# i2Nav-WHU/IC-GVINS

Hardware: NVIDIA H100
Metric: frames/sec (KLT+BA) 1280x560 300-feat 10-KF window (higher is better)
Workload: dtype u8/int32 fixed point + f32 (KLT), f64 (BA)

## Files before the change

### ic_gvins_b200/csrc/ba.cu

```cuda
#include <cooperative_groups.h>
#include <dlfcn.h>
#include <unistd.h>
#include <math.h>
#include <nccl.h>
#include <stdlib.h>
#include <string.h>

#include <algorithm>
#include <string>
#include <thread>
#include <vector>

#include "ba_math.cuh"
#include "common.cuh"
#include "geom_core.cuh"

namespace icg {
using namespace bam;
namespace cg = cooperative_groups;

constexpr int BA_SPLIT_W = 4;
constexpr int BA_CHOL_NB = 8;
constexpr int BA_MARG_MAXB = 72;
constexpr int BA_MAX_NODES = 32;
// ... 259 lines not shown
    __syncthreads();
    if (tid == 0) s_last = atomicAdd(D.vis_cnt + (size_t) w * C.K + rn, 1) == D.ref_nrun[(size_t) w * C.K + rn] - 1;
    __syncthreads();
    if (!s_last) return;
    __threadfence();
    if (tid == 0) D.vis_cnt[(size_t) w * C.K + rn] = 0;
    const int PM = C.K * (C.K - 1), P = D.npairs[w];
    const int *pro = D.pair_ro + (size_t) w * PM, *poff = D.part_off + (size_t) w * (PM + 1);
    for (int p = tid; p < P; p += 128)
        if ((pro[p] >> 8) == rn) {
            atomicAdd(&s_np, 1);
            if (p == 0 || (pro[p - 1] >> 8) != rn) s_p0 = p;
        }
    __syncthreads();
    const double *part = D.gpart + (size_t) w * C.GQ * 210;
    double *Mp = lin_Mp(C, D, b, w);
    for (int p = s_p0 + warp; p < s_p0 + s_np; p += 4) {
        const int k0 = poff[p], k1 = poff[p + 1];
        double acc[7];
#pragma unroll
        for (int j = 0; j < 7; j++) acc[j] = lane + 32 * j < 210 ? __ldcg(part + (size_t) k0 * 210 + lane + 32 * j) : 0.0;
        for (int k = k0 + 1; k < k1; k++) {
            double v[7];
#pragma unroll
            for (int j = 0; j < 7; j++) v[j] = lane + 32 * j < 210 ? __ldcg(part + (size_t) k * 210 + lane + 32 * j) : 0.0;
#pragma unroll
            for (int j = 0; j < 7; j++) acc[j] += v[j];
        }
#pragma unroll
        for (int j = 0; j < 7; j++)
            if (lane + 32 * j < 210) Mp[(size_t) p * 210 + lane + 32 * j] = acc[j];
    }
}


__device__ __forceinline__ void gram2_slots(const BaCaps &C, const BaDev &D, int w, int K, short *s_slot) {
    const int PM = C.K * (C.K - 1), P = D.npairs[w];
    const int *pro = D.pair_ro + (size_t) w * PM;
    for (int e = threadIdx.x; e < K * K; e += blockDim.x) s_slot[e] = -1;
    __syncthreads();
    for (int p = threadIdx.x; p < P; p += blockDim.x) s_slot[(pro[p] >> 8) * K + (pro[p] & 255)] = (short) p;
    __syncthreads();
}
__device__ __forceinline__ double gram2_entry(const BaCaps &C, const BaDev &D, int buf, int w, int K, const short *s_slot, int A, int B) {
    const int P = D.npairs[w];
    const double *Mp = lin_Mp(C, D, buf, w);
    const int bA = A < 6 * K ? A / 6 : K, bB = B < 6 * K ? B / 6 : K;
    const int a = A - 6 * bA, b = B - 6 * bB;
    const int ga = 12 + a, gb = 12 + b;
    double sum = 0;
    if (bA == K) {
        const int idx = tri20(ga, gb);
        double s4[4] = {0, 0, 0, 0};
        int p = 0;
        for (; p + 16 <= P; p += 16) {
            double v[16];
#pragma unroll
            for (int u = 0; u < 16; u++) v[u] = Mp[(size_t) (p + u) * 210 + idx];
#pragma unroll
            for (int u = 0; u < 16; u++) s4[u & 3] += v[u];
        }
        for (; p < P; p++) s4[p & 3] += Mp[(size_t) p * 210 + idx];
        sum = (s4[0] + s4[1]) + (s4[2] + s4[3]);
    } else if (bB == K || bB == bA) {
        const int i1 = tri20(a, bB == K ? gb : b), i2 = tri20(6 + a, bB == K ? gb : 6 + b);
        for (int o0 = 0; o0 < K; o0 += 8) {
            double v1[8], v2[8];
#pragma unroll
            for (int u = 0; u < 8; u++) {
                const int o = o0 + u;
                const int p1 = o < K ? s_slot[bA * K + o] : -1, p2 = o < K ? s_slot[o * K + bA] : -1;
                v1[u] = p1 >= 0 ? Mp[(size_t) p1 * 210 + i1] : 0.0;
                v2[u] = p2 >= 0 ? Mp[(size_t) p2 * 210 + i2] : 0.0;
            }
#pragma unroll
            for (int u = 0; u < 8; u++) sum += v1[u], sum += v2[u];
        }
    } else {
        const int p1 = s_slot[bA * K + bB], p2 = s_slot[bB * K + bA];
        if (p1 >= 0) sum += Mp[(size_t) p1 * 210 + tri20(a, 6 + b)];
        if (p2 >= 0) sum += Mp[(size_t) p2 * 210 + tri20(b, 6 + a)];
    }
    return sum;
}

__device__ __forceinline__ double block_sum(double v, double *s_red);
__device__ __forceinline__ double block_max(double v, double *s_red);
__device__ __forceinline__ double *x_inbox(const BaDev &D, int peer, int w, int from);
__device__ __forceinline__ int tri_idx(int A, int B, int ncv);

__device__ __forceinline__ void schur_store(const BaCaps &C, const BaDev &D, int buf, int w, int K, const short *s_slot, int A, int B, double cw) {
    const int NCV = 6 * K + 7;
    const bool nccl = !D.S.split && D.world > 1;
    if (A == NCV && !nccl) return;
    const size_t e = (size_t) w * C.NS * C.NS + (size_t) B * C.NS + A;
    const double hc = !D.S.split && !nccl && B < NCV ? lin_Hc(C, D, buf, w)[(size_t) B * C.NS + A] : 0.0;
    const double cj = gram2_entry(C, D, buf, w, K, s_slot, A, B);
    if (D.S.split) {
        double *P = x_inbox(D, w % D.world, w, D.rank);
        const int TRI = NCV * (NCV + 1) / 2;
        if (B < NCV) {
            P[tri_idx(A, B, NCV)] = cj - cw;
            if (A == B) P[TRI + A] = cj;
        } else {
            P[TRI + NCV + A] = cj;
            P[TRI + 2 * NCV + A] = cw;
        }
    } else if (nccl) {
        const size_t NN = (size_t) C.NCA * C.NCA;
        double *R = D.red + (size_t) w * (2 * NN + 8);
        R[(size_t) A * C.NCA + B] = R[(size_t) B * C.NCA + A] = cj;
        R[NN + (size_t) A * C.NCA + B] = R[NN + (size_t) B * C.NCA + A] = cw;
    } else {
        double *V = D.visv + (size_t) w * 3 * C.NCV;
        if (B < NCV) {
// ... 427 lines not shown
    const double *part = D.cost_part + (size_t) w * (nblk_vis + 1);
    double cand = 0;
    const int nb = (dm.F + 255) / 256;
    for (int b = 0; b < nb; b++) cand += part[b];
    if (D.rank == 0) cand += part[nblk_vis];
    D.red2[(size_t) w * 4 + 3] = cand;
}

__global__ void __launch_bounds__(256) ba_hsum(BaCaps C, BaDev D) {
    const int w = blockIdx.y;
    if (D.st[w].done) return;
    const int K = D.dims[w].K, NCV = 6 * K + 7, nn = NCV + 1;
    const int NN = C.NCA * C.NCA;
    const int t = blockIdx.x * 256 + threadIdx.x;
    if (t >= nn * nn) return;
    const int A = t / nn, B = t - A * nn;
    if (B < A || B >= NCV) return;
    const double *RED = D.red + (size_t) w * (2 * NN + 8);
    const double cj = RED[(size_t) B * C.NCA + A], cw = RED[NN + (size_t) B * C.NCA + A];
    D.Hs[(size_t) w * C.NS * C.NS + (size_t) B * C.NS + A] = lin_Hc(C, D, 0, w)[(size_t) B * C.NS + A] + (cj - cw);
}

constexpr int SOLVE_THREADS = 256;

__device__ __forceinline__ double block_sum(double v, double *s_red) {
    const int tid = threadIdx.x, lane = tid & 31, warp = tid >> 5;
    for (int o = 16; o > 0; o >>= 1) v += __shfl_down_sync(0xffffffffu, v, o);
    __syncthreads();
    if (lane == 0) s_red[warp] = v;
    __syncthreads();
    double t = 0;
    if (tid == 0) {
        for (int k = 0; k < (int) (blockDim.x >> 5); k++) t += s_red[k];
        s_red[32] = t;
    }
    __syncthreads();
    return s_red[32];
}
__device__ __forceinline__ double block_max(double v, double *s_red) {
    const int tid = threadIdx.x, lane = tid & 31, warp = tid >> 5;
    for (int o = 16; o > 0; o >>= 1) v = fmax(v, __shfl_down_sync(0xffffffffu, v, o));
    __syncthreads();
    if (lane == 0) s_red[warp] = v;
    __syncthreads();
    if (tid == 0) {
        double t = 0;
        for (int k = 0; k < (int) (blockDim.x >> 5); k++) t = fmax(t, s_red[k]);
        s_red[32] = t;
    }
    __syncthreads();
    return s_red[32];
}

__global__ void __launch_bounds__(SOLVE_THREADS, 2) ba_solve(BaCaps C, BaDev D) {
    extern __shared__ double sm[];
    const int w = blockIdx.x, tid = threadIdx.x;
    LmState &st = D.st[w];
    if (st.done) return;
#ifdef ICG_BA_PHASE_CLOCKS
    unsigned long long clk_prev = D.clk ? clock64() : 0ull;
#define SOLVE_CLK(k)                                              \
    if (D.clk && w == 0 && tid == 0) {                            \
        const unsigned long long t_ = clock64();                  \
        atomicAdd(&D.clk[k], t_ - clk_prev), atomicAdd(&D.clk[8 + (k)], 1ull); \
        clk_prev = t_;                                            \
    }
#define SOLVE_CLK_NOW() (D.clk ? clock64() : 0ull)
#define SOLVE_CLK_ADD(k, t0)                                      \
    if (D.clk && w == 0 && tid == 0) atomicAdd(&D.clk[k], clock64() - (t0)), atomicAdd(&D.clk[8 + (k)], 1ull);
#else
#define SOLVE_CLK(k)
#define SOLVE_CLK_NOW() 0ull
#define SOLVE_CLK_ADD(k, t0)
#endif
    const WinDims dm = D.dims[w];
    const int K = dm.K, L = dm.L, NCV = 6 * K + 7, N = 15 * K + 7;
    const int f_first = st.first, f_fresh = st.fresh_lin, f_last = st.last_success, f_iter = st.iter;
    const double f_gmax_old = st.gmax;
    (void) f_gmax_old;
    double *s_red = sm;
    double *s_scale = s_red + 40;
    double *s_g = s_scale + C.NS;
    double *s_rhs = s_g + C.NS;
    double *s_d2 = s_rhs + C.NS;
    double *s_diag = s_d2 + C.NS;
    double *S = s_diag + C.NS;
    const int b = st.lin_buf;
    const double *Hc = lin_Hc(C, D, b, w), *gcam = lin_gc(C, D, b, w), *Hs = D.Hs + (size_t) w * C.NS * C.NS;
    const bool sharded = D.world > 1;
    const int NN = C.NCA * C.NCA;
    const double *RED = D.red + (size_t) w * (2 * NN + 8), *V = D.visv + (size_t) w * 3 * C.NCV;
    auto hvis_diag = [&](int a) { return sharded ? RED[(size_t) a * C.NCA + a] : V[a]; };
    auto g_vis = [&](int a) { return sharded ? RED[(size_t) a * C.NCA + NCV] : V[NCV + a]; };
    auto wphig = [&](int a) { return sharded ? RED[NN + (size_t) a * C.NCA + NCV] : V[2 * NCV + a]; };
    const double camw = D.rank == 0 ? 1.0 : 0.0;
    if (tid == 0 && st.need_lin) st.need_lin = 0;
    double *scale_c = D.scale_c + (size_t) w * C.NS;
    const double *hl = lin_hl(C, D, b, w), *gl = lin_gl(C, D, b, w), *scale_l = D.scale_l + (size_t) w * C.L;

    for (int a = tid; a < N; a += SOLVE_THREADS) {
        double g = gcam[a];
        if (a < NCV) g += g_vis(a);
        s_g[a] = g;
        if (f_first) {
            double h = Hc[(size_t) a * C.NS + a] + (a < NCV ? hvis_diag(a) : 0.0);
            scale_c[a] = 1.0 / (1.0 + sqrt(h));
        }
    }
    __syncthreads();
    for (int a = tid; a < N; a += SOLVE_THREADS) s_scale[a] = scale_c[a];
    double gmax_now = st.gmax;
    if (f_fresh) {
        double c, gml;
        if (sharded) {
            c = RED[2 * NN];
            gml = D.redmax[w];
        } else {
            double cs = 0, gq = 0;
            const double *costf = lin_costf(C, D, b, w);
            for (int f = tid; f < dm.F; f += SOLVE_THREADS) cs += costf[f];
            for (int l = tid; l < L; l += SOLVE_THREADS) gq = fmax(gq, fabs(gl[l]));
            c = block_sum(cs, s_red);
            gml = block_max(gq, s_red);
        }
        double gm = 0;
        for (int a = tid; a < N; a += SOLVE_THREADS) gm = fmax(gm, fabs(s_g[a]));
        gm = fmax(block_max(gm, s_red), gml);
        gmax_now = gm;
        if (tid == 0) {
            st.x_cost = c + st.cost_cam[b];
            st.gmax = gm;
            if (f_first) st.initial_cost = st.x_cost;
            st.fresh_lin = 0;
        }
        __syncthreads();
    }
    if (f_first) {
        __syncthreads();
        if (tid == 0) st.first = 0;
    }
    {
        int term = 0;
        if (f_iter >= st.max_iter) term = 1;
        else if (f_last && gmax_now <= 1e-10) term = 2;
        else if (f_last && st.radius <= 1e-32) term = 2;
        if (term) {
            __syncthreads();
            if (tid == 0) st.done = term, st.step_valid = 0;
            return;
        }
    }
    __syncthreads();
    if (tid == 0) st.iter++;
    const double radius = st.radius;
    SOLVE_CLK(0)

    constexpr bool async_fill = true;
    if (async_fill) {
        for (int i = tid >> 5; i < N; i += SOLVE_THREADS / 32) {
            const double *src = (i < NCV ? Hs : Hc) + (size_t) i * C.NS;
            const unsigned dst = (unsigned) __cvta_generic_to_shared(S + i * (i + 1) / 2);
            for (int j = tid & 31; j <= i; j += 32)
                asm volatile("cp.async.ca.shared.global [%0], [%1], 8;" ::"r"(dst + 8u * j), "l"(src + j) : "memory");
        }
        asm volatile("cp.async.commit_group;" ::: "memory");
    }
    for (int a = tid; a < N; a += SOLVE_THREADS) {
        double h = Hc[(size_t) a * C.NS + a] + (a < NCV ? hvis_diag(a) : 0.0);
        double hs = s_scale[a] * s_scale[a] * h;
        s_d2[a] = fmin(fmax(hs, 1e-6), 1e32) / radius;
        double gw = a < NCV ? wphig(a) : 0.0;
        s_rhs[a] = -s_scale[a] * (s_g[a] - gw);
    }
    if (async_fill) asm volatile("cp.async.wait_all;" ::: "memory");
    __syncthreads();
    if (async_fill) {
        for (int i = tid >> 5; i < N; i += SOLVE_THREADS / 32) {
            double *row = S + i * (i + 1) / 2;
            const double si = s_scale[i];
            for (int j = tid & 31; j <= i; j += 32) {
                double v = si * s_scale[j] * row[j];
                if (i == j) v += s_d2[i];
                row[j] = v;
            }
        }
    } else {
        for (int i = tid >> 5; i < N; i += SOLVE_THREADS / 32) {
            constexpr int MAXQ = 16;
            double hv[MAXQ];
            const int nq = i / 32 + 1;
#pragma unroll
            for (int q = 0; q < MAXQ; q++) {
                const int j = (tid & 31) + 32 * q;
                hv[q] = 0;
                if (q < nq && j <= i) hv[q] = (i < NCV ? Hs : Hc)[(size_t) i * C.NS + j];
            }
#pragma unroll
            for (int q = 0; q < MAXQ; q++) {
                const int j = (tid & 31) + 32 * q;
                if (q < nq && j <= i) {
                    double v = s_scale[i] * s_scale[j] * hv[q];
                    if (i == j) v += s_d2[i];
                    S[i * (i + 1) / 2 + j] = v;
                }
            }
        }
    }
    for (int a = tid; a < N; a += SOLVE_THREADS) S[N * (N + 1) / 2 + a] = s_rhs[a];
    __syncthreads();
    SOLVE_CLK(1)
    __shared__ int s_fail;
    if (tid == 0) s_fail = 0;
    __syncthreads();
    const int NR = N + 1;
    for (int J0 = 0; J0 < N; J0 += BA_CHOL_NB) {
        const int nb = min(BA_CHOL_NB, N - J0);
        const int lane = tid & 31, warp = tid >> 5, g = lane >> 2, kk = lane & 3;
        const int ntile = (NR - J0 + 7) / 8;
        const unsigned long long pc0 = SOLVE_CLK_NOW();
        (void) pc0;
        const int cb = J0 + g;
        const double *rb = S + (cb < NR ? cb * (cb + 1) / 2 : 0);
        const bool okb = cb < NR;
// ... 593 lines not shown
        for (int j = 0; j < 15; j++) Lm[i * 15 + j] = 0.5 * (inv[i * 15 + j] + inv[j * 15 + i]);
    for (int j = 0; j < 15; j++) {
        double d = Lm[j * 15 + j];
        for (int k = 0; k < j; k++) d -= Lm[j * 15 + k] * Lm[j * 15 + k];
        if (!(d > 0)) return false;
        d = sqrt(d);
        Lm[j * 15 + j] = d;
        for (int i = j + 1; i < 15; i++) {
            double s = Lm[i * 15 + j];
            for (int k = 0; k < j; k++) s -= Lm[i * 15 + k] * Lm[j * 15 + k];
            Lm[i * 15 + j] = s / d;
        }
    }
    for (int i = 0; i < 15; i++)
        for (int j = 0; j < 15; j++) U[i * 15 + j] = j >= i ? Lm[j * 15 + i] : 0.0;
    return true;
}

template <typename T>
struct HostDev {
    T *h = nullptr, *d = nullptr;
    size_t n = 0;
    int alloc(size_t count) {
        n = count;
        if (cudaMallocHost(&h, sizeof(T) * count) != cudaSuccess) return ICG_ENOMEM;
        if (cudaMalloc(&d, sizeof(T) * count) != cudaSuccess) return ICG_ENOMEM;
        memset(h, 0, sizeof(T) * count);
        return ICG_OK;
    }
    void release() {
        if (h) cudaFreeHost(h);
        if (d) cudaFree(d);
        h = d = nullptr;
    }
    cudaError_t up(cudaStream_t s, size_t count = 0) { return cudaMemcpyAsync(d, h, sizeof(T) * (count ? count : n), cudaMemcpyHostToDevice, s); }
    cudaError_t down(cudaStream_t s, size_t count = 0) { return cudaMemcpyAsync(h, d, sizeof(T) * (count ? count : n), cudaMemcpyDeviceToHost, s); }
};
}

struct icg_ba {
    BaCaps C;
    BaDev D;
    int device = 0;
    cudaStream_t stream = nullptr;
    cudaStream_t stream_cam = nullptr;
    cudaEvent_t ev_fork = nullptr, ev_join = nullptr;
    bool own_stream = false;
    int nblk_vis = 0;
    int cur_windows = 0;
    int cam_threads = 160;
    size_t smem_cam, smem_solve, smem_schur;
    int ld_schur;
    int use_global_S;
    HostDev<WinDims> dims;
    HostDev<LmState> st;
    HostDev<double> pose, mix, ext, rho, imu_blob, imu_U, gnss_blh, gnss_std, lever, pose_prior, pose_prior_sinfo, mix_prior, mix_prior_std, marg_x0,
        marg_H0, marg_b0, marg_c0;
    HostDev<int> f_meta_s, vb_lm0, ref_nrun;
    HostDev<double> f_const_s;
    HostDev<int> lm_off, lm_perm, lm_fidx, gnss_node, marg_type, marg_node, part_off, pair_ro, vis_ord, npairs;
    HostDev<uint8_t> f_active;
    std::vector<void *> dev_only;
    HostDev<double> scratch;
    HostDev<LmState> st_save;
    HostDev<int> cull_counters;
    void *comm = nullptr;
    double *xbuf = nullptr;
    size_t xbuf_doubles = 0;
    int x_world = 0;
    void *ipc_opened[8] = {nullptr, nullptr, nullptr, nullptr, nullptr, nullptr, nullptr, nullptr};
    unsigned long long epoch = 0;
    size_t smem_solve_cam = 0, smem_step_lm = 0;
    bool solve_cam_stage_a = false;
    bool solve_cam_dsm = false;
    size_t smem_solve_cam_dsm = 0;
    int dsm_variant = 0;
    bool prof = false;
    std::vector<cudaEvent_t> prof_ev;
    std::vector<int> prof_tag;
    size_t prof_used = 0;
    int prof_skip = 1;
    double prof_ms[16] = {0};
    long prof_cnt[16] = {0};
    bool marg_ready = false;
    MargDev M;
    HostDev<int> marg_map;
    HostDev<double> marg_oJ0, marg_oe0, marg_oHp, marg_obp;
};

extern "C" {
static void prof_collect(icg_ba *h);
static void prof_print(icg_ba *h);
}

static int dmalloc(icg_ba *h, double **p, size_t n) {
    if (cudaMalloc(p, sizeof(double) * n) != cudaSuccess) {
        set_error("icg_ba_create: cudaMalloc of %zu doubles failed", n);
        return ICG_ENOMEM;
    }
    cudaMemsetAsync(*p, 0, sizeof(double) * n, h->stream);
    h->dev_only.push_back(*p);
    return ICG_OK;
}

namespace {
struct NcclApi {
// ... 88 lines not shown
    }
    {
        int prio_lo = 0, prio_hi = 0;
        ICG_CUDA(cudaDeviceGetStreamPriorityRange(&prio_lo, &prio_hi));
        ICG_CUDA(cudaStreamCreateWithPriority(&h->stream_cam, cudaStreamNonBlocking, prio_hi));
    }
    ICG_CUDA(cudaEventCreateWithFlags(&h->ev_fork, cudaEventDisableTiming));
    ICG_CUDA(cudaEventCreateWithFlags(&h->ev_join, cudaEventDisableTiming));
    h->prof = getenv("ICG_BA_PROFILE") != nullptr;
    if (getenv("ICG_BA_CAM_THREADS")) h->cam_threads = std::min(CAM_THREADS, std::max(128, atoi(getenv("ICG_BA_CAM_THREADS")) & ~31));
    if (h->prof) {
        double *ck = nullptr;
        if (dmalloc(h, &ck, 48) != ICG_OK) return ICG_ENOMEM;
        h->D.clk = (unsigned long long *) ck;
    }
    if (getenv("ICG_BA_PROFILE_SKIP")) h->prof_skip = atoi(getenv("ICG_BA_PROFILE_SKIP"));
    BaCaps &C = h->C;
    max_L = std::max(1, max_L), max_F = std::max(1, max_F);
    C.NW = max_windows, C.K = max_K, C.L = max_L, C.F = max_F, C.G = std::max(1, max_gnss), C.R = std::max(1, max_marg_r);
    C.NCV = 6 * max_K + 7, C.N = 15 * max_K + 7, C.NS = (C.N + 3) & ~3, C.NCA = 4 * ((C.NCV + 1 + 3) / 4);
    C.RJ = (2 * max_F + 31) & ~31, C.LP = (max_L + 31) & ~31;
    C.NVB = (max_F + 127 - max_K) / (128 - max_K) + max_L / 128 + 4 + max_K;
    C.GQ = std::max(1, std::min(max_F, (C.NVB - 2) * (max_K - 1)));
    h->nblk_vis = (max_F + 255) / 256;
    const size_t NW = max_windows;
#define HD(field, count)                                                       \
    if (h->field.alloc(count) != ICG_OK) {                                     \
        set_error("icg_ba_create: allocation of " #field " failed");           \
        return ICG_ENOMEM;                                                     \
    }
    HD(dims, NW) HD(st, NW) HD(pose, NW * C.K * 7) HD(mix, NW * C.K * 9) HD(ext, NW * 8) HD(rho, NW * C.L)
    HD(imu_blob, NW * C.K * ICG_IMU_BLOB_DOUBLES) HD(imu_U, NW * C.K * 225) HD(gnss_blh, NW * C.G * 3) HD(gnss_std, NW * C.G * 3) HD(lever, NW * 3)
    HD(pose_prior, NW * 7) HD(pose_prior_sinfo, NW * 6) HD(mix_prior, NW * 9) HD(mix_prior_std, NW * 9) HD(marg_x0, NW * BA_MARG_MAXB * 9)
    HD(marg_H0, NW * C.R * C.R) HD(marg_b0, NW * C.R) HD(marg_c0, NW)
    HD(lm_off, NW * (C.L + 1)) HD(lm_perm, NW * C.L) HD(lm_fidx, NW * C.F) HD(gnss_node, NW * C.G) HD(marg_type, NW * BA_MARG_MAXB) HD(marg_node, NW * BA_MARG_MAXB) HD(f_active, NW * C.F)
    HD(scratch, 1024) HD(st_save, NW) HD(cull_counters, 2 * NW) HD(f_meta_s, NW * C.F * 4) HD(vb_lm0, NW * C.NVB) HD(ref_nrun, NW * C.K) HD(f_const_s, NW * C.F * 14)
    HD(part_off, NW * ((size_t) C.K * (C.K - 1) + 1)) HD(pair_ro, NW * (size_t) C.K * (C.K - 1)) HD(vis_ord, NW * C.F) HD(npairs, NW)
#undef HD
    BaDev &D = h->D;
    D.rank = 0, D.world = 1;
    D.dims = h->dims.d, D.st = h->st.d, D.pose = h->pose.d, D.mix = h->mix.d, D.ext = h->ext.d, D.rho = h->rho.d;
    D.f_active = h->f_active.d;
    D.part_off = h->part_off.d, D.pair_ro = h->pair_ro.d, D.vis_ord = h->vis_ord.d, D.npairs = h->npairs.d;
    D.f_meta_s = h->f_meta_s.d, D.vb_lm0 = h->vb_lm0.d, D.ref_nrun = h->ref_nrun.d, D.f_const_s = h->f_const_s.d;
    D.lm_off = h->lm_off.d, D.lm_perm = h->lm_perm.d, D.imu_blob = h->imu_blob.d, D.imu_U = h->imu_U.d;
    D.gnss_node = h->gnss_node.d, D.gnss_blh = h->gnss_blh.d, D.gnss_std = h->gnss_std.d, D.lever = h->lever.d;
    D.pose_prior = h->pose_prior.d, D.pose_prior_sinfo = h->pose_prior_sinfo.d, D.mix_prior = h->mix_prior.d, D.mix_prior_std = h->mix_prior_std.d;
    D.marg_type = h->marg_type.d, D.marg_node = h->marg_node.d, D.marg_x0 = h->marg_x0.d, D.marg_H0 = h->marg_H0.d, D.marg_b0 = h->marg_b0.d, D.marg_c0 = h->marg_c0.d;
    int rc = ICG_OK;
#define DM(field, count) \
    if (rc == ICG_OK) rc = dmalloc(h, &D.field, count);
    DM(pose_c, NW * C.K * 7) DM(mix_c, NW * C.K * 9) DM(ext_c, NW * 8) DM(rho_c, NW * C.L)
    DM(pose_0, NW * C.K * 7) DM(mix_0, NW * C.K * 9) DM(ext_0, NW * 8) DM(rho_0, NW * C.L)
    DM(AW[0], NW * C.NCA * C.LP) DM(Mp[0], NW * (size_t) C.K * (C.K - 1) * 210) DM(visv, NW * 3 * C.NCV)
    DM(gpart, NW * (size_t) C.GQ * 210) DM(costf[0], NW * C.F) DM(hl[0], NW * C.L) DM(gl[0], NW * C.L) DM(scale_l, NW * C.L) DM(scale_c, NW * C.NS)
    DM(Hc[0], NW * C.NS * C.NS) DM(gc[0], NW * C.NS) DM(Hs, NW * C.NS * C.NS) DM(cost_part, NW * (h->nblk_vis + 1)) DM(red, NW * (2 * (size_t) C.NCA * C.NCA + 8)) DM(redmax, NW) DM(red2, NW * 4) DM(step_c, NW * C.NS) DM(step_l, NW * C.L)
#undef DM
    if (rc == ICG_OK) rc = dmalloc(h, &D.gnss_std_0, NW * C.G * 3);
    if (rc == ICG_OK) {
        double *cnt = nullptr;
        rc = dmalloc(h, &cnt, (NW * C.K + 1) / 2);
        D.vis_cnt = (int *) cnt;
    }
    if (rc == ICG_OK) {
        double *fa0 = nullptr;
        rc = dmalloc(h, &fa0, (NW * C.F + 7) / 8 + 1);
        D.f_active_0 = (uint8_t *) fa0;
    }
    if (rc != ICG_OK) return rc;
    h->smem_cam = sizeof(double) * ((size_t) C.K * 480 + (size_t) C.G * 24 + 48 + 16 + 2 * (size_t) C.R + 8) + sizeof(int) * (size_t) C.R + 64;
    size_t vec = sizeof(double) * (40 + 5 * (size_t) C.NS);
    size_t packed = sizeof(double) * ((size_t) (C.N + 1) * (C.N + 2) / 2);
    h->use_global_S = (vec + packed > 220 * 1024) ? 1 : 0;
    h->smem_solve = vec + (h->use_global_S ? 0 : packed);
    D.Sglobal = nullptr;
    memset(&D.S, 0, sizeof(D.S));
    if (h->use_global_S) {
        rc = split_setup(h, 0, 1);
        if (rc != ICG_OK) return rc;
    } else {
        ICG_CUDA(raise_dynamic_smem((const void *) ba_solve, (size_t) (h->smem_solve)));
    }
    h->ld_schur = 16 * ((C.NCA + 15) / 16) + 8;
    h->smem_schur = sizeof(double) * std::max((size_t) SCHUR_RCH * h->ld_schur + SCHUR_RCH, (size_t) SCHUR_PASS * 256);
    ICG_CUDA(raise_dynamic_smem((const void *) ba_schur_dmma, (size_t) (h->smem_schur)));
    ICG_CUDA(cudaFuncSetAttribute(ba_schur_dmma, cudaFuncAttributePreferredSharedMemoryCarveout, cudaSharedmemCarveoutMaxShared));
    ICG_CUDA(raise_dynamic_smem((const void *) ba_lin_cam, (size_t) (h->smem_cam)));
    ICG_CUDA(raise_dynamic_smem((const void *) ba_cost_cam, (size_t) (h->smem_cam)));
    ICG_CUDA(raise_dynamic_smem((const void *) ba_lin_vis, LV_SMEM));
    ICG_CUDA(cudaStreamSynchronize(h->stream));
    h->cur_windows = 0;
    return ICG_OK;
}

void icg_ba_destroy(icg_ba *h) {
    if (!h) return;
    cudaSetDevice(h->device);
    if (h->stream) cudaStreamSynchronize(h->stream);
    prof_collect(h);
    prof_print(h);
    for (cudaEvent_t e : h->prof_ev) cudaEventDestroy(e);
    h->dims.release(), h->st.release(), h->pose.release(), h->mix.release(), h->ext.release(), h->rho.release();
    h->imu_blob.release(), h->imu_U.release(), h->gnss_blh.release(), h->gnss_std.release(), h->lever.release(), h->pose_prior.release();
    h->pose_prior_sinfo.release(), h->mix_prior.release(), h->mix_prior_std.release(), h->marg_x0.release(), h->marg_H0.release(), h->marg_b0.release();
    h->marg_c0.release(), h->lm_off.release(), h->lm_perm.release(), h->lm_fidx.release(), h->gnss_node.release();
    h->f_meta_s.release(), h->vb_lm0.release(), h->ref_nrun.release(), h->f_const_s.release(), h->marg_type.release(), h->marg_node.release(), h->f_active.release(), h->scratch.release(), h->st_save.release(), h->cull_counters.release(), h->part_off.release(), h->pair_ro.release(), h->vis_ord.release(), h->npairs.release();
    if (h->comm) nccl_api().CommDestroy((ncclComm_t) h->comm);
    split_release(h);
    if (h->marg_ready) h->marg_map.release(), h->marg_oJ0.release(), h->marg_oe0.release(), h->marg_oHp.release(), h->marg_obp.release();
    for (void *p : h->dev_only) cudaFree(p);
    if (h->stream_cam) cudaStreamSynchronize(h->stream_cam), cudaStreamDestroy(h->stream_cam);
    if (h->ev_fork) cudaEventDestroy(h->ev_fork);
    if (h->ev_join) cudaEventDestroy(h->ev_join);
    if (h->own_stream && h->stream) cudaStreamDestroy(h->stream);
    delete h;
}

int icg_ba_upload(icg_ba *h, int n, const icg_ba_problem *P) {
    if (!h || !P || n < 1 || n > h->C.NW) {
        set_error("icg_ba_upload: bad arguments (n=%d, capacity %d)", n, h ? h->C.NW : 0);
        return ICG_EINVAL;
    }
    ICG_CUDA(cudaSetDevice(h->device));
    const BaCaps &C = h->C;
#define PK_FAIL(code, ...)                          \
    do {                                            \
        char eb_[512];                              \
        snprintf(eb_, sizeof(eb_), __VA_ARGS__);    \
        err = eb_;                                  \
        return code;                                \
    } while (0)
    auto pack_one = [&](int w, std::string &err) -> int {
        const icg_ba_problem &p = P[w];
        if (p.K < 2 || p.K > C.K || p.L < 0 || p.L > C.L || p.F < 0 || p.F > C.F || p.n_imu < 0 || p.n_imu > p.K - 1 || p.n_gnss < 0 || p.n_gnss > C.G ||
// ... 224 lines not shown
        h->prof_ev.push_back(e);
        h->prof_tag.push_back(0);
    }
    h->prof_tag[h->prof_used] = tag;
    cudaEventRecord(h->prof_ev[h->prof_used++], h->stream);
}
static void prof_collect(icg_ba *h) {
    if (!h->prof) return;
    if (h->prof_used && h->prof_skip > 0) {
        h->prof_skip--;
        h->prof_used = 0;
        return;
    }
    for (size_t i = 1; i < h->prof_used; i++) {
        float ms = 0;
        if (cudaEventElapsedTime(&ms, h->prof_ev[i - 1], h->prof_ev[i]) == cudaSuccess) {
            h->prof_ms[h->prof_tag[i]] += ms;
            h->prof_cnt[h->prof_tag[i]]++;
        }
    }
    h->prof_used = 0;
}
static void prof_print(icg_ba *h) {
    if (!h->prof) return;
    double tot = 0;
    for (int t = 0; t < 16; t++) tot += h->prof_ms[t];
    fprintf(stderr, "[icg_ba profile] handle %p, %d windows: stage totals over all recorded LM sequences (ms, mean us, share)\n", (void *) h, h->cur_windows);
    for (int t = 0; t < 16; t++)
        if (h->prof_cnt[t])
            fprintf(stderr, "  %-28s %9.3f ms  %8.1f us  %5.1f %%\n", PROF_NAMES[t], h->prof_ms[t], 1e3 * h->prof_ms[t] / h->prof_cnt[t], 100.0 * h->prof_ms[t] / tot);
    if (h->D.clk) {
        unsigned long long ck[48];
        if (cudaMemcpy(ck, h->D.clk, sizeof(ck), cudaMemcpyDeviceToHost) == cudaSuccess) {
            static const char *cn[6] = {"factor evaluation", "prior product + cost", "zero H_c", "prior blocks", "IMU J^T J", "GNSS / prior diagonals"};
            fprintf(stderr, "[icg_ba profile] ba_lin_cam phases of window 0 (SM cycles per call, mean):\n");
            for (int k = 0; k < 6; k++)
                if (ck[24 + k]) fprintf(stderr, "  %-28s %9.0f cycles\n", cn[k], (double) ck[16 + k] / (double) ck[24 + k]);
            if (h->D.S.split) {
                static const char *sn_l2[6] = {"per panel: stage B operand", "per panel: warp 0 tile + factor", "per panel: tiles + barrier 1", "per panel: row solve + barrier 2", "whole factorisation", ""};
                static const char *sn_dsm[6] = {"assembly", "per panel: warp 0 tile + factor", "per panel: until block barrier", "per panel: row solve + cl. barrier", "whole factorisation", "backward substitution"};
                const char **sn = h->solve_cam_dsm ? sn_dsm : sn_l2;
                fprintf(stderr, "[icg_ba profile] %s phases of window 0 (SM cycles, mean):\n", h->solve_cam_dsm ? "ba_solve_cam_dsm" : "ba_solve_cam");
                for (int k = 0; k < 6; k++)
                    if (ck[8 + k]) fprintf(stderr, "  %-34s %9.0f cycles\n", sn[k], (double) ck[k] / (double) ck[8 + k]);
                static const char *sn2[5] = {"per panel: wait for the panel column", "(unused)", "per panel: warp 0 diagonal-tile update", "per panel: warp 0 loads + 8x8 factorisation", "per panel: warp 0 write-back"};
                for (int k = 0; k < 5 && h->solve_cam_dsm; k++)
                    if (ck[40 + k]) fprintf(stderr, "  %-50s %9.0f cycles\n", sn2[k], (double) ck[32 + k] / (double) ck[40 + k]);
            }
            static const char *nm[8] = {"gradient / cost / tests", "assembly", "Cholesky", "camera back-substitution", "landmark back-substitution", "candidate + reductions",
                                        "  per panel: warp 0 tile+factor", "  per panel: row solve phase"};
            if (!h->D.S.split) fprintf(stderr, "[icg_ba profile] ba_solve phases of window 0 (SM cycles per call, mean):\n");
            for (int k = 0; k < 8 && !h->D.S.split; k++)
                if (ck[8 + k]) fprintf(stderr, "  %-28s %9.0f cycles\n", nm[k], (double) ck[k] / (double) ck[8 + k]);
        }
    }
}

static int enqueue_lm_split(icg_ba *h, int max_num_iterations);

static int alloc_lin_buf2(icg_ba *h) {
    BaDev &D = h->D;
    if (D.Mp[1]) return ICG_OK;
    const BaCaps &C = h->C;
    const size_t NW = C.NW;
    int rc = ICG_OK;
#define DM(field, count) \
    if (rc == ICG_OK) rc = dmalloc(h, &D.field, count);
    DM(AW[1], NW * C.NCA * C.LP) DM(Mp[1], NW * (size_t) C.K * (C.K - 1) * 210) DM(costf[1], NW * C.F) DM(hl[1], NW * C.L) DM(gl[1], NW * C.L)
    DM(Hc[1], NW * C.NS * C.NS) DM(gc[1], NW * C.NS)
#undef DM
    return rc;
}

static int enqueue_lm(icg_ba *h, int max_num_iterations) {
    if (h->D.S.split) return enqueue_lm_split(h, max_num_iterations);
    if (!h->comm) {
        const int rc = alloc_lin_buf2(h);
        if (rc != ICG_OK) return rc;
    }
    const BaCaps &C = h->C;
    const BaDev &D = h->D;
    const int n = h->cur_windows;
    cudaStream_t s = h->stream;
    const dim3 g_vis(C.NVB - 2, n), g_cost(h->nblk_vis, n);
    static const int cam_fork = getenv("ICG_BA_CAM_FORK") ? atoi(getenv("ICG_BA_CAM_FORK")) : 0;
    auto enqueue_lin = [&](int at_cand) -> int {
        if (cam_fork == 0) {
            ICG_CUDA(cudaEventRecord(h->ev_fork, s));
            ICG_CUDA(cudaStreamWaitEvent(h->stream_cam, h->ev_fork, 0));
            ba_lin_cam<<<n, h->cam_threads, h->smem_cam, h->stream_cam>>>(C, D, at_cand);
            ICG_CUDA(cudaEventRecord(h->ev_join, h->stream_cam));
        }
        prof_mark(h, 0);
        ba_lin_vis<<<g_vis, 128, LV_SMEM, s>>>(C, D, at_cand);
        prof_mark(h, at_cand ? 3 : 1);
        if (cam_fork != 0) {
            ICG_CUDA(cudaEventRecord(h->ev_fork, s));
            ICG_CUDA(cudaStreamWaitEvent(h->stream_cam, h->ev_fork, 0));
            ba_lin_cam<<<n, h->cam_threads, h->smem_cam, h->stream_cam>>>(C, D, at_cand);
            ICG_CUDA(cudaEventRecord(h->ev_join, h->stream_cam));
        }
        if (!h->comm) {
            ICG_CUDA(cudaStreamWaitEvent(s, h->ev_join, 0));
            prof_mark(h, at_cand ? 3 : 6);
        }
        count_launch(2);
        return ICG_OK;
    };
    for (int it = 0; it <= max_num_iterations; it++) {
        if (it == 0 || h->comm) {
            const int rc = enqueue_lin(0);
            if (rc != ICG_OK) return rc;
        }
        ba_schur_dmma<<<dim3(BA_SPLIT_W, n), 256, h->smem_schur, s>>>(C, D, h->ld_schur);
        prof_mark(h, 5);
        if (h->comm) {
            ICG_CUDA(cudaStreamWaitEvent(s, h->ev_join, 0));
            prof_mark(h, 6);
            int rc = nccl_allreduce(h, D.red, (size_t) n * (2 * (size_t) C.NCA * C.NCA + 8), 0);
            if (rc != ICG_OK) return rc;
            rc = nccl_allreduce(h, D.redmax, (size_t) n, 1);
            if (rc != ICG_OK) return rc;
            ba_hsum<<<dim3(((C.NCV + 1) * (C.NCV + 1) + 255) / 256, n), 256, 0, s>>>(C, D);
            prof_mark(h, 12);
        }
        ba_solve<<<n, SOLVE_THREADS, h->smem_solve, s>>>(C, D);
        prof_mark(h, 8);
        count_launch(h->comm ? 3 : 2);
        if (it == max_num_iterations) break;
        if (h->comm) {
            ICG_CUDA(cudaEventRecord(h->ev_fork, s));
            ICG_CUDA(cudaStreamWaitEvent(h->stream_cam, h->ev_fork, 0));
            ba_cost_cam<<<n, h->cam_threads, h->smem_cam, h->stream_cam>>>(C, D, h->nblk_vis);
            ICG_CUDA(cudaEventRecord(h->ev_join, h->stream_cam));
            ba_cost<<<g_cost, 256, 0, s>>>(C, D, h->nblk_vis);
            ICG_CUDA(cudaStreamWaitEvent(s, h->ev_join, 0));
            prof_mark(h, 9);
            ba_pack2<<<(n + 127) / 128, 128, 0, s>>>(C, D, n, h->nblk_vis);
            prof_mark(h, 10);
            int rc = nccl_allreduce(h, D.red2, (size_t) n * 4, 0);
            if (rc != ICG_OK) return rc;
            count_launch(3);
        } else {
            const int rc = enqueue_lin(1);
            if (rc != ICG_OK) return rc;
        }
        ba_accept<<<n, 128, sizeof(double) * 8 * h->nblk_vis, s>>>(C, D);
        prof_mark(h, 11);
        count_launch();
    }
    ICG_CHECK_LAUNCH();
    return ICG_OK;
}

static void split_release(icg_ba *h) {
    for (int r = 0; r < 8; r++)
        if (h->ipc_opened[r]) cudaIpcCloseMemHandle(h->ipc_opened[r]), h->ipc_opened[r] = nullptr;
    if (h->xbuf) cudaFree(h->xbuf), h->xbuf = nullptr;
    if (h->D.S.redv) cudaFree(h->D.S.redv), h->D.S.redv = nullptr;
    if (h->D.S.err) cudaFree(h->D.S.err), h->D.S.err = nullptr;
    if (h->D.S.slm) cudaFree(h->D.S.slm), h->D.S.slm = nullptr;
    if (h->D.S.slm_cnt) cudaFree(h->D.S.slm_cnt), h->D.S.slm_cnt = nullptr;
    if (h->D.Sglobal) cudaFree(h->D.Sglobal), h->D.Sglobal = nullptr;
    h->D.S.split = 0;
}

static int split_setup(icg_ba *h, int rank, int world) {
    if (world < 1 || world > 8 || rank < 0 || rank >= world) {
        set_error("split pipeline: rank %d / world %d out of range (<= 8 GPUs of one box)", rank, world);
        return ICG_EINVAL;
    }
    ICG_CUDA(cudaSetDevice(h->device));
    ICG_CUDA(cudaStreamSynchronize(h->stream));
    split_release(h);
    const BaCaps &C = h->C;
    ShardDev &S = h->D.S;
    const size_t NW = C.NW, G = world;
    const size_t TRI = (size_t) C.NCV * (C.NCV + 1) / 2;
    S.PK = (int) ((TRI + 3 * (size_t) C.NCV + 4 + 3) & ~(size_t) 3);
    S.BS = (SPLIT_HDR + C.NS + 3) & ~3;
    S.RV = (3 * C.NCV + 4 + 3) & ~3;
// ... 820 lines not shown
```

Before: 24280.

## Fuse Schur complement DMMA kernel into ba_solve and drop Hs buffer

Moves the Schur complement SYRK (vision Gram gather plus DMMA reduction over landmark rows) from the separate ba_schur_dmma kernel into a templated ba_solve<true>, writing the reduced camera block directly into shared-memory S instead of through the global Hs/visv buffers. This removes one kernel launch per LM iteration along with the global write and re-read of Hs. The cost is that the Schur work for each window now runs in a single CTA instead of BA_SPLIT_W CTAs, which reduces parallelism. The gram2 pair loop is also rewritten with a predicated tail in place of the scalar remainder loop. An env var keeps the old separate path, and Hs/visv are allocated lazily only for that path.

```diff
diff --git a/ic_gvins_b200/csrc/ba.cu b/ic_gvins_b200/csrc/ba.cu
--- a/ic_gvins_b200/csrc/ba.cu
+++ b/ic_gvins_b200/csrc/ba.cu
@@ -335,15 +335,14 @@
     if (bA == K) {
         const int idx = tri20(ga, gb);
         double s4[4] = {0, 0, 0, 0};
-        int p = 0;
-        for (; p + 16 <= P; p += 16) {
+        for (int p = 0; p < P; p += 16) {
             double v[16];
 #pragma unroll
-            for (int u = 0; u < 16; u++) v[u] = Mp[(size_t) (p + u) * 210 + idx];
-#pragma unroll
-            for (int u = 0; u < 16; u++) s4[u & 3] += v[u];
-        }
-        for (; p < P; p++) s4[p & 3] += Mp[(size_t) p * 210 + idx];
+            for (int u = 0; u < 16; u++) v[u] = p + u < P ? Mp[(size_t) (p + u) * 210 + idx] : 0.0;
+#pragma unroll
+            for (int u = 0; u < 16; u++)
+                if (p + u < P) s4[u & 3] += v[u];
+        }
         sum = (s4[0] + s4[1]) + (s4[2] + s4[3]);
     } else if (bB == K || bB == bA) {
         const int i1 = tri20(a, bB == K ? gb : b), i2 = tri20(6 + a, bB == K ? gb : 6 + b);
@@ -877,8 +876,10 @@
     return s_red[32];
 }
 
+template <bool FUSED>
 __global__ void __launch_bounds__(SOLVE_THREADS, 2) ba_solve(BaCaps C, BaDev D) {
     extern __shared__ double sm[];
+    __shared__ short s_slot[FUSED ? 32 * 32 : 1];
     const int w = blockIdx.x, tid = threadIdx.x;
     LmState &st = D.st[w];
     if (st.done) return;
@@ -915,13 +916,23 @@
     const bool sharded = D.world > 1;
     const int NN = C.NCA * C.NCA;
     const double *RED = D.red + (size_t) w * (2 * NN + 8), *V = D.visv + (size_t) w * 3 * C.NCV;
-    auto hvis_diag = [&](int a) { return sharded ? RED[(size_t) a * C.NCA + a] : V[a]; };
-    auto g_vis = [&](int a) { return sharded ? RED[(size_t) a * C.NCA + NCV] : V[NCV + a]; };
+    auto hvis_diag = [&](int a) { return FUSED ? s_diag[a] : sharded ? RED[(size_t) a * C.NCA + a] : V[a]; };
+    auto g_vis = [&](int a) { return FUSED ? s_rhs[a] : sharded ? RED[(size_t) a * C.NCA + NCV] : V[NCV + a]; };
     auto wphig = [&](int a) { return sharded ? RED[NN + (size_t) a * C.NCA + NCV] : V[2 * NCV + a]; };
     const double camw = D.rank == 0 ? 1.0 : 0.0;
     if (tid == 0 && st.need_lin) st.need_lin = 0;
     double *scale_c = D.scale_c + (size_t) w * C.NS;
     const double *hl = lin_hl(C, D, b, w), *gl = lin_gl(C, D, b, w), *scale_l = D.scale_l + (size_t) w * C.L;
+    if constexpr (FUSED) {
+        gram2_slots(C, D, w, K, s_slot);
+        for (int e = tid; e < 2 * NCV; e += SOLVE_THREADS) {
+            const int a = e < NCV ? e : e - NCV;
+            const double v = gram2_entry(C, D, b, w, K, s_slot, a, e < NCV ? a : NCV);
+            (e < NCV ? s_diag : s_rhs)[a] = v;
+        }
+        __syncthreads();
+        SOLVE_CLK(32)
+    }
 
     for (int a = tid; a < N; a += SOLVE_THREADS) {
         double g = gcam[a];
@@ -980,9 +991,156 @@
     const double radius = st.radius;
     SOLVE_CLK(0)
 
+    if constexpr (FUSED) {
+        const int lane = tid & 31, warp = tid >> 5, g = lane >> 2, kk = lane & 3;
+        const int NCA = 4 * ((NCV + 1 + 3) / 4), T2 = (NCA + 15) / 16, nsuper = T2 * (T2 + 1) / 2, cz = 16 * T2;
+        const int ld = 16 * ((C.NCA + 15) / 16) + 8;
+        const int head = (C.NCV * (C.NCV + 1) / 2 + 1) & ~1;
+        const int rch = min(SCHUR_RCH, (((C.N + 1) * (C.N + 2) / 2 - head) / (2 * (ld + 2))) & ~3);
+        const int bstride = rch * (ld + 2);
+        double *stg = S + head;
+        const double *AW = lin_AW(C, D, b, w);
+        const int nsteps = (L + 3) / 4;
+        auto q_beg = [&](int q) { return 4 * (int) ((long long) nsteps * q / BA_SPLIT_W); };
+        auto q_end = [&](int q) { return min(L, 4 * (int) ((long long) nsteps * (q + 1) / BA_SPLIT_W)); };
+        auto chunk_at = [&](int c, int &r0, int &nr) {
+            for (int q = 0; q < BA_SPLIT_W; q++) {
+                const int n = (q_end(q) - q_beg(q) + rch - 1) / rch;
+                if (c < n) {
+                    r0 = q_beg(q) + c * rch, nr = min(rch, q_end(q) - r0);
+                    return true;
+                }
+                c -= n;
+            }
+            return false;
+        };
+        auto stage = [&](int buf, int r0, int nr) {
+            double *dst = stg + buf * bstride;
+            const int nr4 = (nr + 3) & ~3, hp = NCA / 2;
+            for (int e = tid; e < nr * hp; e += SOLVE_THREADS) {
+                const int rr = e / hp, c = 2 * (e - rr * hp);
+                asm volatile("cp.async.cg.shared.global [%0], [%1], 16;" ::"r"((unsigned) __cvta_generic_to_shared(dst + rr * ld + c)),
+                             "l"(AW + (size_t) (r0 + rr) * C.NCA + c) : "memory");
+            }
+            for (int e = nr * 16 * T2 + tid; e < nr4 * 16 * T2; e += SOLVE_THREADS) dst[e / cz * ld + e % cz] = 0.0;
+            for (int rr = tid; rr < nr; rr += SOLVE_THREADS) {
+                asm volatile("cp.async.ca.shared.global [%0], [%1], 8;" ::"r"((unsigned) __cvta_generic_to_shared(dst + rch * ld + rr)),
+                             "l"(scale_l + r0 + rr) : "memory");
+                asm volatile("cp.async.ca.shared.global [%0], [%1], 8;" ::"r"((unsigned) __cvta_generic_to_shared(dst + rch * (ld + 1) + rr)),
+                             "l"(hl + r0 + rr) : "memory");
+            }
+            asm volatile("cp.async.commit_group;" ::: "memory");
+        };
+        for (int e = tid; e < 2 * rch * (cz - NCA); e += SOLVE_THREADS) {
+            const int rr = e / (cz - NCA);
+            stg[(rr / rch) * bstride + (rr % rch) * ld + NCA + e % (cz - NCA)] = 0.0;
+        }
+        int r0 = 0, nr = 0;
+        const bool any = chunk_at(0, r0, nr);
+        if (any) stage(0, r0, nr);
+        for (int e = tid; e < NCV * (NCV + 1) / 2; e += SOLVE_THREADS) {
+            const int B = (int) ((sqrt(8.0 * e + 1.0) - 1.0) * 0.5);
+            const int Bc = B * (B + 1) / 2 > e ? B - 1 : (B + 1) * (B + 2) / 2 <= e ? B + 1 : B;
+            S[e] = gram2_entry(C, D, b, w, K, s_slot, e - Bc * (Bc + 1) / 2, Bc);
+        }
+        SOLVE_CLK(33)
+        const int npass = (nsuper + SCHUR_PASS - 1) / SCHUR_PASS;
+        int gc = 0;
+        for (int pass = 0; pass < npass; pass++) {
+            int si[2], sj[2];
+            bool on[2];
+#pragma unroll
+            for (int h2 = 0; h2 < 2; h2++) {
+                const int su = (2 * pass + h2) * 8 + warp;
+                on[h2] = su < nsuper;
+                int a = 0, e = on[h2] ? su : 0;
+                while (e >= T2 - a) e -= T2 - a, a++;
+                si[h2] = a, sj[h2] = a + e;
+            }
+            double tot[2][4][2];
+#pragma unroll
+            for (int h2 = 0; h2 < 2; h2++)
+#pragma unroll
+                for (int q = 0; q < 4; q++) tot[h2][q][0] = tot[h2][q][1] = 0;
+            int ci = 0;
+            for (int q = 0; q < BA_SPLIT_W; q++) {
+                double acc[2][4][2];
+#pragma unroll
+                for (int h2 = 0; h2 < 2; h2++)
+#pragma unroll
+                    for (int u = 0; u < 4; u++) acc[h2][u][0] = acc[h2][u][1] = 0;
+                for (int rq = q_beg(q); rq < q_end(q); rq += rch, ci++, gc++) {
+                    const int nrc = min(rch, q_end(q) - rq), nr4 = (nrc + 3) & ~3;
+                    __syncthreads();
+                    int r1, n1;
+                    if (chunk_at(ci + 1, r1, n1) || (pass + 1 < npass && chunk_at(0, r1, n1))) stage((gc + 1) & 1, r1, n1);
+                    else asm volatile("cp.async.commit_group;" ::: "memory");
+                    asm volatile("cp.async.wait_group 1;" ::: "memory");
+                    __syncthreads();
+                    double *rows = stg + (gc & 1) * bstride, *sphi = rows + rch * ld;
+                    for (int rr = tid; rr < nr4; rr += SOLVE_THREADS) {
+                        double ph = 0;
+                        if (rr < nrc) {
+                            const double sl = sphi[rr], hs = sl * sl * sphi[rch + rr];
+                            ph = sl * sl / (hs + fmin(fmax(hs, 1e-6), 1e32) / radius);
+                        }
+                        sphi[rr] = ph;
+                    }
+                    __syncthreads();
+                    for (int ks = 0; ks < nr4 / 4; ks++) {
+                        const double *row = rows + (4 * ks + kk) * ld;
+                        const double ph = sphi[4 * ks + kk];
+#pragma unroll
+                        for (int h2 = 0; h2 < 2; h2++) {
+                            if (!on[h2]) continue;
+                            const double xb0 = row[16 * sj[h2] + g], xb1 = row[16 * sj[h2] + 8 + g];
+                            const double a0 = row[16 * si[h2] + g] * ph, a1 = row[16 * si[h2] + 8 + g] * ph;
+                            dmma884(acc[h2][0][0], acc[h2][0][1], a0, xb0);
+                            dmma884(acc[h2][1][0], acc[h2][1][1], a0, xb1);
+                            dmma884(acc[h2][2][0], acc[h2][2][1], a1, xb0);
+                            dmma884(acc[h2][3][0], acc[h2][3][1], a1, xb1);
+                        }
+                    }
+                }
+#pragma unroll
+                for (int h2 = 0; h2 < 2; h2++)
+#pragma unroll
+                    for (int u = 0; u < 4; u++) tot[h2][u][0] += acc[h2][u][0], tot[h2][u][1] += acc[h2][u][1];
+            }
+            __syncthreads();
+            double hc[2][4][2];
+#pragma unroll
+            for (int h2 = 0; h2 < 2; h2++)
+#pragma unroll
+                for (int u = 0; u < 4; u++)
+#pragma unroll
+                    for (int e = 0; e < 2; e++) {
+                        const int r = 16 * si[h2] + 8 * (u >> 1) + g, cc = 16 * sj[h2] + 8 * (u & 1) + 2 * kk + e;
+                        hc[h2][u][e] = on[h2] && r <= cc && cc < NCV ? Hc[(size_t) cc * C.NS + r] : 0.0;
+                    }
+#pragma unroll
+            for (int h2 = 0; h2 < 2; h2++)
+#pragma unroll
+                for (int u = 0; u < 4; u++)
+#pragma unroll
+                    for (int e = 0; e < 2; e++) {
+                        const int r = 16 * si[h2] + 8 * (u >> 1) + g, cc = 16 * sj[h2] + 8 * (u & 1) + 2 * kk + e;
+                        if (!on[h2] || r > cc || r >= NCV) continue;
+                        const double cw = tot[h2][u][e];
+                        if (cc < NCV) {
+                            double &v = S[cc * (cc + 1) / 2 + r];
+                            v = hc[h2][u][e] + (v - cw);
+                        } else if (cc == NCV) {
+                            s_rhs[r] = -s_scale[r] * (s_g[r] - cw);
+                        }
+                    }
+        }
+        __syncthreads();
+        SOLVE_CLK(34)
+    }
     constexpr bool async_fill = true;
     if (async_fill) {
-        for (int i = tid >> 5; i < N; i += SOLVE_THREADS / 32) {
+        for (int i = (FUSED ? NCV : 0) + (tid >> 5); i < N; i += SOLVE_THREADS / 32) {
             const double *src = (i < NCV ? Hs : Hc) + (size_t) i * C.NS;
             const unsigned dst = (unsigned) __cvta_generic_to_shared(S + i * (i + 1) / 2);
             for (int j = tid & 31; j <= i; j += 32)
@@ -994,6 +1152,7 @@
         double h = Hc[(size_t) a * C.NS + a] + (a < NCV ? hvis_diag(a) : 0.0);
         double hs = s_scale[a] * s_scale[a] * h;
         s_d2[a] = fmin(fmax(hs, 1e-6), 1e32) / radius;
+        if (FUSED && a < NCV) continue;
         double gw = a < NCV ? wphig(a) : 0.0;
         s_rhs[a] = -s_scale[a] * (s_g[a] - gw);
     }
@@ -1693,6 +1852,7 @@
     size_t smem_cam, smem_solve, smem_schur;
     int ld_schur;
     int use_global_S;
+    bool separate_schur = false;
     HostDev<WinDims> dims;
     HostDev<LmState> st;
     HostDev<double> pose, mix, ext, rho, imu_blob, imu_U, gnss_blh, gnss_std, lever, pose_prior, pose_prior_sinfo, mix_prior, mix_prior_std, marg_x0,
@@ -1887,9 +2047,9 @@
     if (rc == ICG_OK) rc = dmalloc(h, &D.field, count);
     DM(pose_c, NW * C.K * 7) DM(mix_c, NW * C.K * 9) DM(ext_c, NW * 8) DM(rho_c, NW * C.L)
     DM(pose_0, NW * C.K * 7) DM(mix_0, NW * C.K * 9) DM(ext_0, NW * 8) DM(rho_0, NW * C.L)
-    DM(AW[0], NW * C.NCA * C.LP) DM(Mp[0], NW * (size_t) C.K * (C.K - 1) * 210) DM(visv, NW * 3 * C.NCV)
+    DM(AW[0], NW * C.NCA * C.LP) DM(Mp[0], NW * (size_t) C.K * (C.K - 1) * 210)
     DM(gpart, NW * (size_t) C.GQ * 210) DM(costf[0], NW * C.F) DM(hl[0], NW * C.L) DM(gl[0], NW * C.L) DM(scale_l, NW * C.L) DM(scale_c, NW * C.NS)
-    DM(Hc[0], NW * C.NS * C.NS) DM(gc[0], NW * C.NS) DM(Hs, NW * C.NS * C.NS) DM(cost_part, NW * (h->nblk_vis + 1)) DM(red, NW * (2 * (size_t) C.NCA * C.NCA + 8)) DM(redmax, NW) DM(red2, NW * 4) DM(step_c, NW * C.NS) DM(step_l, NW * C.L)
+    DM(Hc[0], NW * C.NS * C.NS) DM(gc[0], NW * C.NS) DM(cost_part, NW * (h->nblk_vis + 1)) DM(red, NW * (2 * (size_t) C.NCA * C.NCA + 8)) DM(redmax, NW) DM(red2, NW * 4) DM(step_c, NW * C.NS) DM(step_l, NW * C.L)
 #undef DM
     if (rc == ICG_OK) rc = dmalloc(h, &D.gnss_std_0, NW * C.G * 3);
     if (rc == ICG_OK) {
@@ -1914,7 +2074,15 @@
         rc = split_setup(h, 0, 1);
         if (rc != ICG_OK) return rc;
     } else {
-        ICG_CUDA(raise_dynamic_smem((const void *) ba_solve, (size_t) (h->smem_solve)));
+        ICG_CUDA(raise_dynamic_smem((const void *) ba_solve<true>, (size_t) (h->smem_solve)));
+        ICG_CUDA(raise_dynamic_smem((const void *) ba_solve<false>, (size_t) (h->smem_solve)));
+    }
+    h->separate_schur = getenv("ICG_BA_SEPARATE_SCHUR") && atoi(getenv("ICG_BA_SEPARATE_SCHUR")) == 1;
+    if (h->prof && !h->use_global_S) {
+        int nb = 0;
+        ICG_CUDA(cudaOccupancyMaxActiveBlocksPerMultiprocessor(&nb, h->separate_schur ? ba_solve<false> : ba_solve<true>, SOLVE_THREADS, h->smem_solve));
+        fprintf(stderr, "[icg_ba profile] ba_solve<%s>: %d CTAs per SM (%zu B dynamic shared memory)\n", h->separate_schur ? "separate" : "fused", nb,
+                h->smem_solve);
     }
     h->ld_schur = 16 * ((C.NCA + 15) / 16) + 8;
     h->smem_schur = sizeof(double) * std::max((size_t) SCHUR_RCH * h->ld_schur + SCHUR_RCH, (size_t) SCHUR_PASS * 256);
@@ -2245,6 +2413,9 @@
             if (!h->D.S.split) fprintf(stderr, "[icg_ba profile] ba_solve phases of window 0 (SM cycles per call, mean):\n");
             for (int k = 0; k < 8 && !h->D.S.split; k++)
                 if (ck[8 + k]) fprintf(stderr, "  %-28s %9.0f cycles\n", nm[k], (double) ck[k] / (double) ck[8 + k]);
+            static const char *nf[3] = {"gather: diag H_vis, g_vis", "gather: vision Gram entries", "Schur SYRK + epilogue"};
+            for (int k = 0; k < 3 && !h->D.S.split; k++)
+                if (ck[40 + k]) fprintf(stderr, "  %-28s %9.0f cycles\n", nf[k], (double) ck[32 + k] / (double) ck[40 + k]);
         }
     }
 }
@@ -2265,7 +2436,22 @@
     return rc;
 }
 
+static int alloc_hs(icg_ba *h) {
+    BaDev &D = h->D;
+    const BaCaps &C = h->C;
+    const size_t NW = C.NW;
+    int rc = ICG_OK;
+    if (!D.Hs) rc = dmalloc(h, &D.Hs, NW * C.NS * C.NS);
+    if (rc == ICG_OK && !D.visv && !D.S.split && !h->comm) rc = dmalloc(h, &D.visv, NW * 3 * C.NCV);
+    return rc;
+}
+
 static int enqueue_lm(icg_ba *h, int max_num_iterations) {
+    const bool fused = !h->D.S.split && !h->comm && !h->separate_schur;
+    if (!fused) {
+        const int rc = alloc_hs(h);
+        if (rc != ICG_OK) return rc;
+    }
     if (h->D.S.split) return enqueue_lm_split(h, max_num_iterations);
     if (!h->comm) {
         const int rc = alloc_lin_buf2(h);
@@ -2305,21 +2491,27 @@
             const int rc = enqueue_lin(0);
             if (rc != ICG_OK) return rc;
         }
-        ba_schur_dmma<<<dim3(BA_SPLIT_W, n), 256, h->smem_schur, s>>>(C, D, h->ld_schur);
-        prof_mark(h, 5);
-        if (h->comm) {
-            ICG_CUDA(cudaStreamWaitEvent(s, h->ev_join, 0));
-            prof_mark(h, 6);
-            int rc = nccl_allreduce(h, D.red, (size_t) n * (2 * (size_t) C.NCA * C.NCA + 8), 0);
-            if (rc != ICG_OK) return rc;
-            rc = nccl_allreduce(h, D.redmax, (size_t) n, 1);
-            if (rc != ICG_OK) return rc;
-            ba_hsum<<<dim3(((C.NCV + 1) * (C.NCV + 1) + 255) / 256, n), 256, 0, s>>>(C, D);
-            prof_mark(h, 12);
-        }
-        ba_solve<<<n, SOLVE_THREADS, h->smem_solve, s>>>(C, D);
-        prof_mark(h, 8);
-        count_launch(h->comm ? 3 : 2);
+        if (fused) {
+            ba_solve<true><<<n, SOLVE_THREADS, h->smem_solve, s>>>(C, D);
+            prof_mark(h, 8);
+            count_launch();
+        } else {
+            ba_schur_dmma<<<dim3(BA_SPLIT_W, n), 256, h->smem_schur, s>>>(C, D, h->ld_schur);
+            prof_mark(h, 5);
+            if (h->comm) {
+                ICG_CUDA(cudaStreamWaitEvent(s, h->ev_join, 0));
+                prof_mark(h, 6);
+                int rc = nccl_allreduce(h, D.red, (size_t) n * (2 * (size_t) C.NCA * C.NCA + 8), 0);
+                if (rc != ICG_OK) return rc;
+                rc = nccl_allreduce(h, D.redmax, (size_t) n, 1);
+                if (rc != ICG_OK) return rc;
+                ba_hsum<<<dim3(((C.NCV + 1) * (C.NCV + 1) + 255) / 256, n), 256, 0, s>>>(C, D);
+                prof_mark(h, 12);
+            }
+            ba_solve<false><<<n, SOLVE_THREADS, h->smem_solve, s>>>(C, D);
+            prof_mark(h, 8);
+            count_launch(h->comm ? 3 : 2);
+        }
         if (it == max_num_iterations) break;
         if (h->comm) {
             ICG_CUDA(cudaEventRecord(h->ev_fork, s));
```

Result: no change. 24330 (median of 6 runs) (+0.2%).
